# gotaku6629/CTC

Hardware: AMD Instinct MI355X
Metric: ctc_samples_per_sec (higher is better)
Workload: dtype f32; 1 GPU; NoBlankCTC B=256 T=150 C=158 S<=20 fp32 (BASELINE configs[1]); variant=noblank, per_gpu_batch=256, global_batch=256, T=150, C=158, S=20, parallelism=dp1 (batch-sharded), launch=graph, graph_steps=50, step=fused loss+grad launch + scale_grad launch (loss.backward(), grad_out=1)

## Files before the change

ctc_amd/csrc/common.hpp:

```cpp
#pragma once
#include <hip/hip_runtime.h>
#include <stdint.h>

#if !defined(CTC_AMD_EXPERIMENTS) &&                                                                            \
    (defined(CTC_X_NOSTATUS) || defined(CTC_X_NOREDUCE) || defined(CTC_X_NORETURN) || defined(CTC_X_NOCHAIN) || \
     defined(CTC_X_NOPRIO) || defined(CTC_X_NOREAD) || defined(CTC_X_NOWRITE) ||                                 \
     defined(CTC_X_WMASK) || defined(CTC_X_NOPROG) || defined(CTC_X_NORENORM) ||                                \
     defined(CTC_X_ROWDPP) || defined(CTC_X_SCALAR_STEP) || defined(CTC_X_NO_POOL_GATHER) || defined(CTC_X_FLOW_NO_GPRIO) || defined(CTC_X_FLOW_NOEXP) || defined(CTC_X_FLOW_NO_DELEGATE) || defined(CTC_X_FLOW_DELEGATE_OWN) || \
     defined(CTC_FLOW_TILE_WAVES))
#error "CTC_X_* experiment switches need -DCTC_AMD_EXPERIMENTS (A/B builds only, never the product library)"
#endif

namespace ctc {

constexpr int kWave = 64;
constexpr float kNeg = -10000000000000.0f;
constexpr float kInfeasible = 1.0e12f;

struct LaneStates { int K, SP; };
inline LaneStates lane_states(int S)
{
    int K = 1;
    while (K <= 4 && S > kWave * K) K *= 2;
    return {K, (S + K - 1) / K * K};
}

__device__ __forceinline__ int lane_id() { return threadIdx.x & (kWave - 1); }
__device__ __forceinline__ int wave_id() { return __builtin_amdgcn_readfirstlane(threadIdx.x >> 6); }

__device__ __forceinline__ void stream_store(float *p, float v) { __builtin_nontemporal_store(v, p); }
__device__ __forceinline__ void stream_store(float4 *p, float4 v)
{
    typedef float native4 __attribute__((ext_vector_type(4)));
    native4 n = {v.x, v.y, v.z, v.w};
    __builtin_nontemporal_store(n, reinterpret_cast<native4 *>(p));
}

typedef float wt_f2 __attribute__((ext_vector_type(2)));
typedef float wt_f4 __attribute__((ext_vector_type(4)));
__device__ __forceinline__ void through_store(wt_f2 *p, wt_f2 v)
{
    asm volatile("global_store_dwordx2 %0, %1, off sc1" ::"v"(p), "v"(v) : "memory");
}
__device__ __forceinline__ void through_store(wt_f4 *p, wt_f4 v)
{
    asm volatile("global_store_dwordx4 %0, %1, off sc1\n\ts_nop 1" ::"v"(p), "v"(v) : "memory");
}
typedef unsigned wt_u2 __attribute__((ext_vector_type(2)));
__device__ __forceinline__ void through_store(wt_u2 *p, wt_u2 v)
{
    asm volatile("global_store_dwordx2 %0, %1, off sc1" ::"v"(p), "v"(v) : "memory");
}
__device__ __forceinline__ void through_store(unsigned *p, unsigned v)
{
    asm volatile("global_store_dword %0, %1, off sc1" ::"v"(p), "v"(v) : "memory");
}
template <bool NT, typename V, int A = 8>
__device__ __forceinline__ void grad_store(V *p, V v)
{
    if (NT) {
        typedef V __attribute__((aligned(A))) VA;
        __builtin_nontemporal_store(v, reinterpret_cast<VA *>(p));
    } else {
        through_store(p, v);
    }
}

constexpr unsigned kStatusNoblankStarved = 1u, kStatusBinaryStarved = 2u, kStatusBlankStarved = 4u;
constexpr unsigned kStatusAlignStarved = 8u;
__device__ __forceinline__ void raise_status(unsigned *counter, unsigned bit)
{
#ifdef CTC_X_NOSTATUS
    return;
#endif
    if (lane_id() == 0) __hip_atomic_fetch_or(counter + 2, bit, __ATOMIC_RELAXED, __HIP_MEMORY_SCOPE_AGENT);
}

constexpr int kGateWord = 11;
__device__ __forceinline__ unsigned *arrival_shard(unsigned *counter, int sh) { return counter + 64 + 4 * sh + 2; }
__device__ __forceinline__ bool gate_on(const unsigned *counter)
{
    typedef const __attribute__((address_space(4))) unsigned const_u32;
    return *(const_u32 *)(uintptr_t)(counter + kGateWord) != 0;
}
__device__ __forceinline__ void note_arrival(unsigned *counter, int b)
{
    if (!gate_on(counter)) return;
    __hip_atomic_fetch_add(arrival_shard(counter, b & 15), 1u, __ATOMIC_RELAXED, __HIP_MEMORY_SCOPE_AGENT);
}
__device__ __forceinline__ void reset_arrivals(unsigned *counter)
{
    for (int sh = 0; sh < 16; ++sh) __hip_atomic_store(arrival_shard(counter, sh), 0u, __ATOMIC_RELAXED, __HIP_MEMORY_SCOPE_AGENT);
}

#ifdef CTC_AMD_DIAGNOSTICS
#define CTC_DIAG(p) ((p).stop)
#else
#define CTC_DIAG(p) 0
#endif

__device__ __forceinline__ void lds_order() { asm volatile("" ::: "memory"); }

__device__ __forceinline__ int opaque_v(int x) { asm volatile("" : "+v"(x)); return x; }
__device__ __forceinline__ int opaque_s(int x) { asm volatile("" : "+s"(x)); return x; }

__device__ __forceinline__ int xcd_sample(int bid, int B)
{
    const int x = bid & 7, k = bid >> 3, q = B >> 3, r = B & 7;
    return x * q + (x < r ? x : r) + k;
}

__device__ __forceinline__ float wave_shr1(float v, float fill)
{
    return __builtin_bit_cast(float, __builtin_amdgcn_update_dpp(
        __builtin_bit_cast(int, fill), __builtin_bit_cast(int, v), 0x138, 0xf, 0xf, false));
}
__device__ __forceinline__ float wave_shl1(float v, float fill)
// ... 299 lines not shown
```

ctc_amd/csrc/noblank.hip:

```cpp
#include <type_traits>

#include "lattice.hpp"
#include "launch.hpp"

namespace ctc {

struct NoblankParams {
    const float *x;
    int64_t st, sb;
    const void *lab;
    int lab64;
    const int64_t *in_len, *tgt_len;
    int T, B, C, S, SP;
    int stop;
    float loss_scale, grad_scale;
    float *nll, *loss, *grad;
    float *gamma;
    float *lattice;
    int64_t slab;
    unsigned *counter;
    int next_round;
    float ls_a, ls_b;
    int koff;
};
// ... 472 lines not shown
            pl.next_round = (q.B > cus && (size_t)q.T * ((q.C * 4 + 127) / 128) <= (size_t)kKmWorkers * kWave) ? cus : 0;
            return pl;
        }
#endif
        pl.family = kNoblankR16;
        pl.next_round = (q.B > cus && (size_t)q.T * ((q.C * esz + 127) / 128) <= (size_t)kPipeWorkers * kWave) ? cus : 0;
        pl.ps = q.B > 2 * cus && cus > 0 && !q.sw.no_ps && q.want_grad && 4 * n4 + 2 * n2 <= 12;
        if (pl.ps) pl.grid = cus;
        return pl;
    }
    if (r16_only || (z.glb && z.smem > kMaxLds)) return NoblankPlan{};
    if (fast) {
        pl.ch = (q.C + kWave - 1) / kWave;
        pl.dual = q.B > cus && 2 * z.smem <= kMaxLds;
        const size_t xsmem = xr_smem_bytes(q.T, z.SP, q.C);
        const bool xr = !q.sw.no_xr && xsmem <= kMaxLds && (!pl.dual || 2 * xsmem <= kMaxLds);
        pl.family = xr ? kNoblankXr : kNoblankPipelined;
        pl.lds = xr ? xsmem : z.smem;
        return pl;
    }
    pl.family = kNoblankFused;
    pl.K = z.K; pl.glb = z.glb;
    pl.ch = q.C <= 256 && !z.glb ? (q.C + kWave - 1) / kWave : 0;
    pl.lds = z.smem;
    return pl;
}

template <int N, int... Ns, typename F>
static int with_constant(int n, F f)
{
    if constexpr (sizeof...(Ns) == 0) {
        return f(std::integral_constant<int, N>());
    } else {
        return n == N ? f(std::integral_constant<int, N>()) : with_constant<Ns...>(n, f);
    }
}
template <typename F>
static int with_row_chunks(int n4, int n2, F f)
{
    return with_constant<1, 2, 4, 5, 6, 8, 9, 10, 12, 13, 14, 16>(4 * n4 + n2, [&](auto k) {
        return f(std::integral_constant<int, decltype(k)::value / 4>(), std::integral_constant<int, decltype(k)::value % 4>());
    });
}

static int noblank_launch(const NoblankPlan &pl, int dtype, NoblankParams &p, hipStream_t s)
{
    const dim3 grid(pl.grid), block(kThreads);
    p.next_round = pl.next_round; p.koff = pl.koff;
    switch (pl.family) {
        case kNoblankR16:
            return with_row_chunks(pl.n4, pl.n2, [&](auto n4, auto n2) {
                return with_constant<0, 1>(pl.nt, [&](auto nt) {
                    return with_constant<CTC_AMD_BF16, CTC_AMD_F16, CTC_AMD_F32>(dtype, [&](auto dt) {
                        using E = std::conditional_t<decltype(dt)::value == CTC_AMD_BF16, __bf16,
                                                     std::conditional_t<decltype(dt)::value == CTC_AMD_F16, _Float16, float>>;
                        constexpr int A = decltype(n4)::value, Bq = decltype(n2)::value;
                        constexpr bool NT = decltype(nt)::value != 0;
                        if constexpr (4 * A + 2 * Bq <= 12)
                            if (pl.ps) return launch<noblank_r16_kernel<A, Bq, NT, true, E>>(grid, block, pl.lds, s, p);
                        return launch<noblank_r16_kernel<A, Bq, NT, false, E>>(grid, block, pl.lds, s, p);
                    });
                });
            });
#ifdef CTC_AMD_DIAGNOSTICS
        case kNoblankKm:
            return with_row_chunks(pl.n4, pl.n2, [&](auto n4, auto n2) {
                return with_constant<0, 1>(pl.nt, [&](auto nt) {
                    return launch<noblank_km_kernel<decltype(n4)::value, decltype(n2)::value, decltype(nt)::value != 0>>(
                        grid, block, pl.lds, s, p);
                });
            });
#endif
        case kNoblankXr:
        case kNoblankPipelined:
            return with_constant<1, 2, 3, 4>(pl.ch, [&](auto ch) {
                return with_constant<0, 1>(pl.dual, [&](auto dual) {
                    constexpr int CH = decltype(ch)::value;
                    constexpr bool DUAL = decltype(dual)::value != 0;
                    return pl.family == kNoblankXr ? launch<noblank_xr_kernel<CH, DUAL>>(grid, block, pl.lds, s, p)
                                                   : launch<noblank_pipelined_kernel<CH, DUAL>>(grid, block, pl.lds, s, p);
                });
            });
        case kNoblankFused:
            return with_constant<1, 2, 4>(pl.K, [&](auto k) {
                constexpr int K = decltype(k)::value;
                if (pl.glb) return launch<noblank_fused_kernel<K, 0, true>>(grid, block, pl.lds, s, p);
                return with_constant<1, 2, 3, 4, 0>(pl.ch, [&](auto ch) {
                    return launch<noblank_fused_kernel<K, decltype(ch)::value>>(grid, block, pl.lds, s, p);
                });
            });
        default: return CTC_AMD_ERR_UNSUPPORTED_SHAPE;
    }
}

static int noblank_run(const void *x, int64_t stride_t, int64_t stride_b,
                       const void *labels, int labels_i64,
                       const int64_t *in_len, const int64_t *tgt_len,
                       int T, int B, int C, int S,
                       float loss_scale, float grad_scale,
                       float *nll, float *loss, void *grad,
                       void *workspace, void *stream, float label_smoothing, int x_dtype = CTC_AMD_F32,
                       float *gamma = nullptr)
{
    const NoblankSwitches sw = gamma ? NoblankSwitches{} : noblank_switches();
    NoblankParams p;
    if (const int rc = noblank_params(p, x, stride_t, stride_b, labels, labels_i64, in_len, tgt_len, T, B, C, S, loss_scale,
                                      grad_scale, nll, loss, grad, gamma, workspace, label_smoothing, sw))
        return rc;
    const NoblankQuery q = {T, B, C, S, x_dtype, stride_t, stride_b,
                            (unsigned)(reinterpret_cast<uintptr_t>(x) & 15), (unsigned)(reinterpret_cast<uintptr_t>(grad) & 15),
                            p.grad != nullptr, gamma != nullptr, label_smoothing >= 0.f,
                            device_cus(),
                            sw};
// ... 120 lines not shown
```

ctc_amd/csrc/noblank_km.hpp:

```cpp
#pragma once
#include "noblank_km_asm.hpp"

namespace ctc {

constexpr int kKmWorkers = 12, kKmG = 4;
constexpr int kKmPad = 8;
constexpr float kKmMinLog2 = -4096.f;
constexpr float kKmSink = -8388608.f;
constexpr float kKmNone = -16777216.f;
constexpr int kKmIntMin = -2147483647 - 1;
constexpr int kKmKprog = kKmWorkers, kKmMprog = kKmWorkers + 2;

__host__ __device__ inline int km_pitch_c(int T)
{
    int tp = T + 2 * kKmPad;
    while ((tp & 3) != 2) ++tp;
    return tp;
}
__host__ __device__ inline int km_pitch_m(int T)
{
    int tp = T + 2 * kKmPad;
    while ((tp & 7) != 4) ++tp;
    return tp;
}
// ... 603 lines not shown
        if (CTC_DIAG(p) < 0) stamp(p, 3 + (G - 1 - g) < 6 ? 3 + (G - 1 - g) : 5);
        if (first) { asm volatile("" ::"v"(prefetched)); first = false; }
        int occn[2] = {0, 0}, max_occ = 0;
        if (need_a > 0) {
            occn[0] = own[0] ? sm.occ[lst[0]] : 0;
            occn[1] = own[1] ? sm.occ[lst[1]] : 0;
            max_occ = __builtin_amdgcn_readfirstlane(sm.occ[(p.SP + 3) & ~3]);
        }
        const Row &x = v[g];
        const int t = tv[g];
        const bool live = t >= 0 && t < Tlive;
        float pr[2];
        int ks[2];
#pragma unroll
        for (int s = 0; s < 2; ++s) {
            const bool in = live && own[s];
            const int offc = in ? lst[s] * sm.TPc + t : p.SP * sm.TPc, offm = in ? lst[s] * sm.TPm + t : p.SP * sm.TPm;
            const float a = sm.ma[offm], bq = sm.mb[offm];
            const int ca = cell_k(sm.ka[offc]);
            const int kbq = __builtin_bit_cast(int, sm.kb[offc].x);
            const float pm = in ? sm.em[offc].x : 1.f;
            pr[s] = in ? a * bq * __builtin_amdgcn_rcpf(pm) : 0.f;
            ks[s] = ca + kbq;
        }
        if (__builtin_amdgcn_ballot_w64(live && !have_ref) != 0) {
            int km = max(pr[0] > 0.f ? ks[0] : kKmIntMin, pr[1] > 0.f ? ks[1] : kKmIntMin);
            row16_allmax(km);
            if (live && !have_ref && km != kKmIntMin) { kref = km; have_ref = true; }
        }
        float z[2];
#pragma unroll
        for (int s = 0; s < 2; ++s) z[s] = pr[s] > 0.f ? __builtin_amdgcn_ldexpf(pr[s], ks[s] - kref) : 0.f;
        float tot = z[0] + z[1];
        row16_allsum(tot);
        float rinv = (live && tot > 0.f) ? -gsc * p.ls_a * __builtin_amdgcn_rcpf(tot) : 0.f;
        if (starved) {
            rinv = __builtin_nanf("");
            raise_status(p.counter, kStatusNoblankStarved);
        }
        Row::zero_tile(trow, i16);
        lds_order();
#pragma unroll
        for (int s = 0; s < 2; ++s)
            if (own[s] && occn[s] == 0) *gat[s] = z[s] * rinv;
        for (int k = 1; k <= max_occ; ++k) {
            lds_order();
#pragma unroll
            for (int s = 0; s < 2; ++s)
                if (own[s] && occn[s] == k) *gat[s] += z[s] * rinv;
        }
        lds_order();
        if (t >= 0) {
            float *gp = p.grad + ((int64_t)t * p.B + b) * p.C;
            if (smooth) x.template store_grad<NT, true>(gp, trow, i16, rs[g] * (1.f - p.ls_b), col_ok, live ? -p.ls_b * gsc : 0.f);
            else x.template store_grad<NT, false>(gp, trow, i16, rs[g], col_ok, 0.f);
        }
        lds_order();
    }
    stamp(p, 7);
}

}
```

ctc_amd/csrc/noblank_r16.hpp:

```cpp
#pragma once

namespace ctc {

typedef float f2_t __attribute__((ext_vector_type(2)));

#define CTC_ROW16(OP)                                                                   \
    "s_nop 1\n\t" OP " %0, %0, %0 quad_perm:[1,0,3,2] row_mask:0xf bank_mask:0xf\n\t"   \
    "s_nop 1\n\t" OP " %0, %0, %0 quad_perm:[2,3,0,1] row_mask:0xf bank_mask:0xf\n\t"   \
    "s_nop 1\n\t" OP " %0, %0, %0 row_half_mirror row_mask:0xf bank_mask:0xf\n\t"       \
    "s_nop 1\n\t" OP " %0, %0, %0 row_mirror row_mask:0xf bank_mask:0xf\n\t"            \
    "s_nop 1"
__device__ __forceinline__ void row16_allmax(float &v) { asm volatile(CTC_ROW16("v_max_f32_dpp") : "+v"(v)); }
__device__ __forceinline__ void row16_allsum(float &v) { asm volatile(CTC_ROW16("v_add_f32_dpp") : "+v"(v)); }
__device__ __forceinline__ void row16_allmax(int &v) { asm volatile(CTC_ROW16("v_max_i32_dpp") : "+v"(v)); }

constexpr int kR16Pad = 2 * kPrefetch + 1;
#ifndef CTC_R16_BLOCK
#define CTC_R16_BLOCK 16
#endif
constexpr int kR16Block = CTC_R16_BLOCK;
__host__ __device__ inline int r16_pitch(int T)
{
    int tp = T + 2 * kR16Pad + 1;
    while ((tp & 3) != 2) ++tp;
    return tp;
}

__device__ __forceinline__ int r16_row(int T, int u, int g, int k)
{
    const int H = (T + 1) >> 1, idx = 2 * kPipeWorkers * g + 2 * u + (k >> 1);
    if ((k & 1) == 0) return idx < H ? idx : -1;
    return idx < T - H ? T - 1 - idx : -1;
}

struct R16Smem {
    int TP;
    cell_t *em, *al, *be;
    float *dummy, *stage, *cs;
    int *cnt, *lab, *occ, *done;
    __device__ R16Smem(float *base, int T, int SP, int RP)
    {
        TP = r16_pitch(T);
        cell_t *lat = reinterpret_cast<cell_t *>(base);
        em = lat + kR16Pad;
        al = em + (size_t)(SP + 1) * TP;
        be = al + (size_t)(SP + 1) * TP;
        dummy = reinterpret_cast<float *>(lat + (size_t)3 * (SP + 1) * TP);
        cnt = reinterpret_cast<int *>(dummy + 8);
        lab = cnt + 16;
        occ = lab + ((SP + 3) & ~3);
        cs = reinterpret_cast<float *>(occ + ((SP + 3) & ~3) + 4);
        done = reinterpret_cast<int *>(cs + 4 * kPipeWorkers);
        stage = cs + 64;
// ... 141 lines not shown
        if (have < G) wait_upto(i + kR16Block - 1 + kPrefetch);
        if (CTC_DIAG(p) < 0) stamp(p, 2 + i / 16);
#ifndef CTC_X_NORENORM
        renorm();
#endif
#pragma unroll
        for (int q = 0; q < kPairs; ++q) {
            const pair_t e = ring[q & 1];
#ifndef CTC_X_NOREAD
            ring[q & 1] = rb[FWD ? q : kPairs - 1 - q];
#endif
#ifdef CTC_X_NOWRITE
            const pair_t o = step2(e, q == 0);
            if (q == kPairs - 1) wb[0] = o;
#elif defined(CTC_X_WMASK)
            const pair_t o = step2(e, q == 0);
            if (lane < SP) wb[FWD ? q : kPairs - 1 - q] = o;
#else
            wb[FWD ? q : kPairs - 1 - q] = step2(e, q == 0);
#endif
        }
        rb += D * kPairs;
        wb += D * kPairs;
    }
    if (CTC_DIAG(p) == -77 && lane == 0)
        reinterpret_cast<unsigned long long *>(p.counter)[FWD ? 0 : 1] = __builtin_amdgcn_s_memtime() - loop_t0;
    lds_order();
    *prog = i;
    if (have < G) wait_upto(Tb - 1);
    renorm();
    static_assert(kPrefetch == 4, "tail groups assume one ring revolution of two pairs");
    if (!FWD) { rb += kPairs - 2; wb += kPairs - 2; }
    for (; i < Tb; i += kPrefetch) {
#pragma unroll
        for (int q = 0; q < 2; ++q) {
            const pair_t e = ring[q];
            ring[q] = rb[FWD ? q : 1 - q];
            wb[FWD ? q : 1 - q] = step2(e, q == 0);
        }
        rb += D * 2;
        wb += D * 2;
    }
    lds_order();
    *prog = Tb;
    __builtin_amdgcn_s_setprio(0);
    cell_t fin = (FWD ? sm.al : sm.be)[(size_t)(L - 1) * sm.TP + (FWD ? Tb - 1 : 0)];
    if (starved) {
        raise_status(p.counter, kStatusNoblankStarved);
        fin = make_cell(__builtin_nanf(""), 0);
    }
    return fin;
}

typedef float f4_t __attribute__((ext_vector_type(4)));
typedef float f4u_t __attribute__((ext_vector_type(4), aligned(8)));

typedef unsigned u2a4_t __attribute__((ext_vector_type(2), aligned(4)));
template <typename E>
__device__ __forceinline__ f2_t r16_widen2(unsigned u)
{
    if constexpr (__is_same(E, __bf16)) {
        const f2_t f = {__builtin_bit_cast(float, u << 16), __builtin_bit_cast(float, u & 0xffff0000u)};
        return f;
    } else {
        typedef _Float16 h2_t __attribute__((ext_vector_type(2)));
        return __builtin_convertvector(__builtin_bit_cast(h2_t, u), f2_t);
    }
}
template <typename E>
__device__ __forceinline__ unsigned r16_narrow2(f2_t v)
{
    typedef E e2_t __attribute__((ext_vector_type(2)));
    return __builtin_bit_cast(unsigned, __builtin_convertvector(v, e2_t));
}

template <bool kRaw, int N4, int N2>
struct R16RawRegs {};
template <int N4, int N2>
struct R16RawRegs<true, N4, N2> {
    wt_u2 ra[N4 > 0 ? N4 : 1];
    unsigned rc[N2 > 0 ? N2 : 1];
};

template <int N4, int N2, typename E = float>
struct R16Row : R16RawRegs<sizeof(E) == 2, N4, N2> {
    static constexpr bool kLowp = sizeof(E) == 2;
    f4_t a[N4 > 0 ? N4 : 1];
    f2_t c[N2 > 0 ? N2 : 1];
    static constexpr int kCols = 64 * N4 + 32 * N2;
    static constexpr bool kLast4 = N2 == 0;
    __device__ static __forceinline__ int off4(int j, int i16) { return 64 * j + 4 * i16; }
    __device__ static __forceinline__ int off2(int k, int i16) { return 64 * N4 + 32 * k + 2 * i16; }
    __device__ static __forceinline__ int off_last(int i16) { return kLast4 ? off4(N4 - 1, i16) : off2(N2 - 1, i16); }

    __device__ __forceinline__ void load(const E *row, int i16, int c_last)
    {
        if constexpr (kLowp) {
#pragma unroll
            for (int j = 0; j < N4; ++j)
                this->ra[j] = *reinterpret_cast<const u2a4_t *>(row + ((kLast4 && j == N4 - 1) ? c_last : off4(j, i16)));
#pragma unroll
            for (int k = 0; k < N2; ++k)
                this->rc[k] = *reinterpret_cast<const unsigned *>(row + (k == N2 - 1 ? c_last : off2(k, i16)));
        } else {
#pragma unroll
            for (int j = 0; j < N4; ++j)
// ... 37 lines not shown
            const float q = (a[j].x + a[j].y) + (a[j].z + a[j].w);
            s += ((kLast4 && j == N4 - 1) && !valid_last) ? 0.f : q;
        }
#pragma unroll
        for (int k = 0; k < N2; ++k) s += (k == N2 - 1 && !valid_last) ? 0.f : c[k].x + c[k].y;
        return s;
    }
    __device__ __forceinline__ float exp_sum(float mb, float mbl)
    {
        const f2_t l2 = {kLog2e, kLog2e};
        f2_t acc = {0.f, 0.f};
#pragma unroll
        for (int j = 0; j < N4; ++j) {
            const float b = (kLast4 && j == N4 - 1) ? mbl : mb;
            const f2_t bb = {b, b};
            f2_t lo = {a[j].x, a[j].y}, hi = {a[j].z, a[j].w};
            lo = __builtin_elementwise_fma(lo, l2, bb);
            hi = __builtin_elementwise_fma(hi, l2, bb);
            a[j].x = __builtin_amdgcn_exp2f(lo.x);
            a[j].y = __builtin_amdgcn_exp2f(lo.y);
            a[j].z = __builtin_amdgcn_exp2f(hi.x);
            a[j].w = __builtin_amdgcn_exp2f(hi.y);
            const f2_t e0 = {a[j].x, a[j].y}, e1 = {a[j].z, a[j].w};
            acc += e0;
            acc += e1;
        }
#pragma unroll
        for (int k = 0; k < N2; ++k) {
            const float b = k == N2 - 1 ? mbl : mb;
            const f2_t bb = {b, b};
            const f2_t lo = __builtin_elementwise_fma(c[k], l2, bb);
            c[k].x = __builtin_amdgcn_exp2f(lo.x);
            c[k].y = __builtin_amdgcn_exp2f(lo.y);
            acc += c[k];
        }
        return acc.x + acc.y;
    }
    __device__ __forceinline__ void to_tile(float *trow, int i16) const
    {
#pragma unroll
        for (int j = 0; j < N4; ++j) *reinterpret_cast<f4_t *>(trow + off4(j, i16)) = a[j];
#pragma unroll
        for (int k = 0; k < N2; ++k) *reinterpret_cast<f2_t *>(trow + off2(k, i16)) = c[k];
    }
    __device__ static __forceinline__ void zero_tile(float *trow, int i16)
    {
        const f4_t z4 = {0.f, 0.f, 0.f, 0.f};
        const f2_t z2 = {0.f, 0.f};
#pragma unroll
        for (int j = 0; j < N4; ++j) *reinterpret_cast<f4_t *>(trow + off4(j, i16)) = z4;
#pragma unroll
        for (int k = 0; k < N2; ++k) *reinterpret_cast<f2_t *>(trow + off2(k, i16)) = z2;
    }
    template <bool NT, bool LS>
    __device__ __forceinline__ void store_grad(E *g, const float *trow, int i16, float rs, bool col_ok, float cb) const
    {
        const f2_t r2 = {rs, rs}, cb2 = {cb, cb};
        f4_t o4[N4 > 0 ? N4 : 1];
        f2_t o2[N2 > 0 ? N2 : 1];
#pragma unroll
        for (int j = 0; j < N4; ++j) o4[j] = *reinterpret_cast<const f4_t *>(trow + off4(j, i16));
#pragma unroll
        for (int k = 0; k < N2; ++k) o2[k] = *reinterpret_cast<const f2_t *>(trow + off2(k, i16));
#pragma unroll
        for (int j = 0; j < N4; ++j) {
            const f4_t o = o4[j];
            f2_t olo = {o.x, o.y}, ohi = {o.z, o.w};
            if (LS) { olo += cb2; ohi += cb2; }
            const f2_t xlo = {a[j].x, a[j].y}, xhi = {a[j].z, a[j].w};
            const f2_t vlo = __builtin_elementwise_fma(xlo, r2, olo), vhi = __builtin_elementwise_fma(xhi, r2, ohi);
            if (!(kLast4 && j == N4 - 1) || col_ok) {
                if constexpr (kLowp) {
                    const wt_u2 n = {r16_narrow2<E>(vlo), r16_narrow2<E>(vhi)};
                    grad_store<NT, wt_u2, 4>(reinterpret_cast<wt_u2 *>(g + off4(j, i16)), n);
                } else {
                    const f4_t v = {vlo.x, vlo.y, vhi.x, vhi.y};
                    grad_store<NT>(reinterpret_cast<f4_t *>(g + off4(j, i16)), v);
                }
            }
        }
#pragma unroll
        for (int k = 0; k < N2; ++k) {
            f2_t o = o2[k];
            if (LS) o += cb2;
            const f2_t v = __builtin_elementwise_fma(c[k], r2, o);
            if (k < N2 - 1 || col_ok) {
                if constexpr (kLowp) grad_store<NT, unsigned, 4>(reinterpret_cast<unsigned *>(g + off2(k, i16)), r16_narrow2<E>(v));
                else grad_store<NT>(reinterpret_cast<f2_t *>(g + off2(k, i16)), v);
            }
        }
    }
    __device__ __forceinline__ void touch() const
    {
        if constexpr (kLowp) {
#pragma unroll
            for (int j = 0; j < N4; ++j) asm volatile("" ::"v"(this->ra[j]));
#pragma unroll
            for (int k = 0; k < N2; ++k) asm volatile("" ::"v"(this->rc[k]));
        } else {
#pragma unroll
            for (int j = 0; j < N4; ++j) asm volatile("" ::"v"(a[j]));
#pragma unroll
            for (int k = 0; k < N2; ++k) asm volatile("" ::"v"(c[k]));
        }
    }
    template <bool NT>
    __device__ static __forceinline__ void store_zero(E *g, int i16, bool col_ok)
    {
        if constexpr (kLowp) {
            const wt_u2 z4 = {0u, 0u};
#pragma unroll
            for (int j = 0; j < N4; ++j)
                if (!(kLast4 && j == N4 - 1) || col_ok) grad_store<NT, wt_u2, 4>(reinterpret_cast<wt_u2 *>(g + off4(j, i16)), z4);
#pragma unroll
            for (int k = 0; k < N2; ++k)
                if (k < N2 - 1 || col_ok) grad_store<NT, unsigned, 4>(reinterpret_cast<unsigned *>(g + off2(k, i16)), 0u);
            return;
        }
        const f4_t z4 = {0.f, 0.f, 0.f, 0.f};
        const f2_t z2 = {0.f, 0.f};
#pragma unroll
        for (int j = 0; j < N4; ++j)
            if (!(kLast4 && j == N4 - 1) || col_ok) grad_store<NT>(reinterpret_cast<f4_t *>(g + off4(j, i16)), z4);
#pragma unroll
        for (int k = 0; k < N2; ++k)
            if (k < N2 - 1 || col_ok) grad_store<NT>(reinterpret_cast<f2_t *>(g + off2(k, i16)), z2);
    }
};

static bool r16_shape(int C, int &n4, int &n2)
{
    if (C < 2 || C > 256 || (C & 1)) return false;
    const int U = (C + 31) / 32;
    if (U & 1) { n4 = U / 2; n2 = 1; }
    else if ((C & 3) == 0) { n4 = U / 2; n2 = 0; }
    else { n4 = U / 2 - 1; n2 = 2; }
    return true;
}

template <typename E>
__device__ __forceinline__ const E *r16_xrow(const NoblankParams &p, int t, int b)
{
    return reinterpret_cast<const E *>(p.x) + (int64_t)t * p.st + (int64_t)b * p.sb;
}
template <int N4, int N2, bool NT, bool PS = false, typename E = float>
__global__ __launch_bounds__(kThreads, 4) void noblank_r16_kernel(NoblankParams p)
{
    extern __shared__ float4 smem_raw[];
    typedef R16Row<N4, N2, E> Row;
    constexpr int RP = Row::kCols;
    constexpr int G = kPipeRows / 4;
    const R16Smem sm(reinterpret_cast<float *>(smem_raw), p.T, p.SP, RP);
    const int tid = threadIdx.x, w = wave_id(), lane = lane_id();
    int vb = blockIdx.x;
    int b = xcd_sample(vb, p.B);
    if (tid == 64 * kChainB) note_arrival(p.counter, b);
    const int u = (w == 0 || w == kChainB) ? -1 : (w < kChainB ? w - 1 : w - 2);
    const int rho = lane >> 4, i16 = lane & 15;

    if (CTC_DIAG(p) == 1) return;
    stamp(p, 0);
    stamp_setup(p, 0);
    auto spread = [&](int which) {
        if (CTC_DIAG(p) != -50 || w != 1 || lane != 0) return;
        const int bid = blockIdx.x, nb = gridDim.x;
        const int slot = bid == 0 ? 0 : bid == nb / 2 ? 2 : bid == nb - 1 ? 4 : -1;
        if (slot < 0) return;
        unsigned long long *o = reinterpret_cast<unsigned long long *>(p.counter) + 8 + 2 * (slot + which);
        o[0] = __builtin_amdgcn_s_memtime();
        o[1] = __builtin_amdgcn_s_memrealtime();
    };
    spread(0);
    ScalarLengths len(p.in_len + b, p.tgt_len + b);
    int tv0[G];
    Row v[G];
#ifdef CTC_R16_NX
    constexpr int NX = PS ? CTC_R16_NX : 0;
#else
    constexpr int NX = PS ? (NT ? 2 : 3) : 0;
#endif
    Row nx[NX > 0 ? NX : 1];
    const bool col_ok = Row::off_last(i16) < p.C;
    const int c_last = col_ok ? Row::off_last(i16) : p.C - (Row::kLast4 ? 4 : 2);
    const int Hh = (p.T + 1) >> 1;
    bool grp[G];
#pragma unroll
    for (int g = 0; g < G; ++g) grp[g] = u >= 0 && 2 * kPipeWorkers * g + 2 * u < Hh;
    int klab = 0;
    if (PS && w == 0 && lane < p.S) klab = load_label(p.lab, p.lab64, (int64_t)b * p.S + lane);
    if (u >= 0) {
#pragma unroll
        for (int g = 0; g < G; ++g) {
            tv0[g] = r16_row(p.T, u, g, rho);
            if (g >= NX) v[g].load(r16_xrow<E>(p, tv0[g] >= 0 ? tv0[g] : 0, b), i16, c_last);
            else nx[g].load(r16_xrow<E>(p, tv0[g] >= 0 ? tv0[g] : 0, b), i16, c_last);
        }
        stamp_setup(p, 1);
        if (PS) {
#pragma unroll
            for (int g = 0; g < G; ++g) {
// ... 43 lines not shown
        if ((vb - (int)blockIdx.x) / (int)gridDim.x < 6) stamp_mode(p, -400, (vb - (int)blockIdx.x) / (int)gridDim.x);
        return CTC_DIAG(p) != 2;
    };
    auto advance = [&]() -> bool {
        stamp_mode(p, -300, (vb - (int)blockIdx.x) / (int)gridDim.x);
        if ((vb - (int)blockIdx.x) / (int)gridDim.x < 6) stamp_mode(p, -400, 6 + (vb - (int)blockIdx.x) / (int)gridDim.x);
        if (!more) return false;
        vb = vbn;
        b = bn;
        len = len_n;
        klab = klab_n;
        asm volatile("s_waitcnt lgkmcnt(0)\n\ts_barrier" ::: "memory");
        return true;
    };
    auto chain_sample = [&](const NoblankParams &p, const int lane) {
    const R16Smem sm(reinterpret_cast<float *>(smem_raw), p.T, p.SP, RP);
    if (Tb == 0) {
        if (w == 0)
            publish_and_reduce_sum(-kNeg, b, p.B, p.nll, p.loss, p.loss_scale, p.counter);
        return;
    }
    {
        __builtin_amdgcn_s_setprio(3);
        if (w == 0) {
            const cell_t a = r16_chain<true>(p, sm, p.T, Tb, L, p.SP, lane);
            stamp(p, 11);
            bool late = false;
            {
                int spins = 0;
                while (*(lds_cvint *)sm.done < kPipeWorkers) {
                    if (++spins >= kSpinLimit) { late = true; break; }
                    __builtin_amdgcn_s_sleep(2);
                }
                lds_order();
            }
            const float csum = wave_sum(lane < 4 * kPipeWorkers ? sm.cs[lane] : 0.f);
            const float am = a.x;
            float nll = am > 0.f ? -(__builtin_amdgcn_logf(am) + (float)(cell_k(a) - kXrBias) + csum) * kLn2 : -kNeg;
            if (am != am) nll = am;
            if (late) {
                raise_status(p.counter, kStatusNoblankStarved);
                nll = __builtin_nanf("");
            }
            publish_and_reduce_sum(nll, b, p.B, p.nll, p.loss, p.loss_scale, p.counter);
            if (CTC_DIAG(p) == -50 && lane == 0) {
                const int bid = blockIdx.x, nb = gridDim.x;
                const int slot = bid == 0 ? 6 : bid == nb / 2 ? 7 : bid == nb - 1 ? 8 : -1;
                if (slot >= 0) {
                    unsigned long long *o = reinterpret_cast<unsigned long long *>(p.counter) + 8 + 2 * slot;
                    o[0] = __builtin_amdgcn_s_memtime();
                    o[1] = __builtin_amdgcn_s_memrealtime();
                }
            }
        } else if (p.grad || p.gamma) {
            r16_chain<false>(p, sm, p.T, Tb, L, p.SP, lane);
            stamp(p, 11);
        }
    }
    };

    auto worker_sample = [&](const NoblankParams &p, const int lane, const int u) {
    const R16Smem sm(reinterpret_cast<float *>(smem_raw), p.T, p.SP, RP);
    const int rho = lane >> 4, i16 = lane & 15;
    int tv[G];
#pragma unroll
    for (int g = 0; g < G; ++g) tv[g] = PS ? opaque_v(tv0[g]) : tv0[g];
    const bool has_grad = PS || p.grad != nullptr, has_gamma = !PS && !Row::kLowp && p.gamma != nullptr;
    auto load_next = [&]() {
        if (!PS) return;
#pragma unroll
        for (int g = 0; g < NX; ++g) nx[g].load(r16_xrow<E>(p, tv[g] >= 0 ? tv[g] : 0, bn), i16, c_last);
    };
#define CTC_R16_RELOAD(g)                                                                             \
    do {                                                                                              \
        if (PS && (g) >= NX) v[g].load(r16_xrow<E>(p, tv[g] >= 0 ? tv[g] : 0, bn), i16, c_last); \
    } while (0)
    if (!PS && Tb == 0) {
        if (p.grad) {
#pragma unroll
            for (int g = 0; g < G; ++g)
                if (tv[g] >= 0) Row::template store_zero<NT>(reinterpret_cast<E *>(p.grad) + ((int64_t)tv[g] * p.B + b) * p.C, i16, col_ok);
        }
        if (!Row::kLowp && p.gamma) {
#pragma unroll
            for (int g = 0; g < G; ++g)
                for (int l = i16; l < p.S && tv[g] >= 0; l += 16) p.gamma[((int64_t)b * p.T + tv[g]) * p.S + l] = 0.f;
        }
        return;
    }
    float *tile = sm.stage + (size_t)u * 4 * RP;
    float *trow = tile + rho * RP;
    int lst[2];
    float *gat[2];
#pragma unroll
    for (int s = 0; s < 2; ++s) {
        lst[s] = 16 * s + i16;
        gat[s] = trow + (lst[s] < p.SP ? sm.lab[lst[s]] : 0);
    }
    const bool own[2] = {lst[0] < L, lst[1] < L};
    const bool smooth = p.ls_b != 0.f;
    cell_t *const spare_w = reinterpret_cast<cell_t *>(sm.dummy);
    float mrow[G];
#pragma unroll
    for (int g = 0; g < G; ++g) {
        if (g == 0) __builtin_amdgcn_s_setprio(2);
        else __builtin_amdgcn_s_setprio(1);
        if (g < NX) v[g] = nx[g];
        if (grp[g]) {
            Row &x = v[g];
            x.widen();
            const int t = tv[g];
            const bool live = t >= 0 && t < Tb;
            float m = x.max();
            row16_allmax(m);
            mrow[g] = m;
            if (CTC_DIAG(p) < 0 && g == 0) stamp(p, 6);
            x.to_tile(trow, i16);
            lds_order();
            float xv[2];
#pragma unroll
            for (int s = 0; s < 2; ++s) xv[s] = *gat[s];
            lds_order();
#pragma unroll
            for (int s = 0; s < 2; ++s) {
                const float ec = (xv[s] - m) * kLog2e;
                const float e2 = fmaxf(smooth ? p.ls_a * ec : ec, kXrMinLog2);
                const float fl = __builtin_floorf(e2);
                const float pm = __builtin_amdgcn_exp2f(e2 - fl);
                cell_t *dst = (live && lst[s] < p.SP) ? sm.em + lst[s] * sm.TP + t : spare_w;
                *dst = own[s] ? make_cell(pm, (int)fl) : zero;
            }
            lds_order();
        } else {
            mrow[g] = 0.f;
        }
        sm.cnt[u] = 4 * (g + 1);
        __builtin_amdgcn_sched_barrier(0);
        if (CTC_DIAG(p) < 0) stamp(p, 8 + g);
    }
    __builtin_amdgcn_s_setprio(0);
    load_next();
    float rs[G];
    float cacc = 0.f;
#pragma unroll
    for (int g = 0; g < G; ++g) {
        rs[g] = 0.f;
        if (!grp[g]) continue;
        Row &x = v[g];
        const int t = tv[g];
        const bool live = t >= 0 && t < Tb;
        const float m = mrow[g];
        float sx = 0.f;
        if (smooth) {
            sx = x.sum(col_ok);
            row16_allsum(sx);
        }
        const float mb = -m * kLog2e;
        float sum = x.exp_sum(mb, col_ok ? mb : ninf);
        row16_allsum(sum);
        const float l2sum = __builtin_amdgcn_logf(sum);
        rs[g] = live ? p.grad_scale * __builtin_amdgcn_rcpf(sum) : 0.f;
        const float cst = smooth ? __builtin_fmaf(p.ls_b, __builtin_fmaf(sx - (float)p.C * m, kLog2e, -(float)p.C * l2sum), -p.ls_a * l2sum)
                                 : -l2sum;
        cacc += live ? cst : 0.f;
    }
    if (i16 == 0) sm.cs[4 * u + rho] = cacc;
    lds_order();
    if (lane == 0) __hip_atomic_fetch_add(sm.done, 1, __ATOMIC_RELAXED, __HIP_MEMORY_SCOPE_WORKGROUP);
    stamp(p, 2);
    if (u == kPipeWorkers - 1 && has_grad) {
        const int kl = lane < p.SP ? sm.lab[lane] : -1;
        int oc = 0;
        for (int l2 = 0; l2 < L; ++l2) {
            const int q = __builtin_amdgcn_readlane(kl, l2);
            oc += (l2 < lane && q == kl) ? 1 : 0;
        }
        if (lane >= L) oc = 0;
        int mo = 0;
        while (__builtin_amdgcn_ballot_w64(oc > mo) != 0) ++mo;
        if (lane < p.SP) sm.occ[lane] = oc;
        sm.occ[(p.SP + 3) & ~3] = mo;
        lds_order();
        sm.occ[((p.SP + 3) & ~3) + 1] = 1;
    }
    float prefetched = 0.f;
    if (!PS && p.next_round > 0 && (int)blockIdx.x + p.next_round < p.B) {
        const int nb = xcd_sample(blockIdx.x + p.next_round, p.B);
        const int line = u * kWave + lane;
        const int lines_per_row = (p.C * (int)sizeof(E) + 127) / 128;
        const int t = line / lines_per_row, c = (line - t * lines_per_row) * (128 / (int)sizeof(E));
        typedef const E __attribute__((address_space(1))) gelem;
        if (t < p.T) prefetched = (float)*(gelem *)(r16_xrow<E>(p, t, nb) + (c < p.C ? c : p.C - 1));
    }
    if (!has_grad && !has_gamma) return;

    const int Tlive = Tb;
    const float gsc = p.grad_scale;
    Row::zero_tile(trow, i16);
    lds_order();
    if (PS) {
#pragma unroll
        for (int g = 0; g < NX; ++g) nx[g].touch();
    }
    int need_a_[G], need_b_[G];
#pragma unroll
    for (int g = 0; g < G; ++g) {
        need_a_[g] = 0;
        need_b_[g] = 0;
#pragma unroll
        for (int k = 0; k < 4; ++k) {
            const int tk = r16_row(p.T, u, g, k);
            if (tk >= 0 && tk < Tlive) {
                need_a_[g] = max(need_a_[g], tk + 1);
                need_b_[g] = max(need_b_[g], Tlive - tk);
            }
        }
    }
    int crow[2];
#pragma unroll
    for (int s = 0; s < 2; ++s) crow[s] = opaque_v((lst[s] < p.SP ? lst[s] : p.SP) * sm.TP);
    E *grow[G];
#pragma unroll
    for (int g = 0; g < G; ++g) {
        grow[g] = reinterpret_cast<E *>(p.grad) + ((int64_t)(tv[g] > 0 ? tv[g] : 0) * p.B + b) * p.C;
        asm volatile("" : "+v"(grow[g]));
    }
    bool starved = false;

    int kref = 0;
    bool have_ref = false;
    int occn[2] = {0, 0}, max_occ = 0;
    if (has_grad) {
        int spins = 0;
        while (*(lds_cvint *)(sm.occ + ((p.SP + 3) & ~3) + 1) == 0) {
            if (++spins >= kSpinLimit) { starved = true; break; }
            __builtin_amdgcn_s_sleep(2);
        }
        lds_order();
        occn[0] = own[0] ? sm.occ[lst[0]] : 0;
        occn[1] = own[1] ? sm.occ[lst[1]] : 0;
        max_occ = __builtin_amdgcn_readfirstlane(sm.occ[(p.SP + 3) & ~3]);
    }
    const bool first_occ[2] = {own[0] && occn[0] == 0, own[1] && occn[1] == 0};
    float *const sink = sm.dummy + 4;
#pragma unroll
    for (int g = G - 1; g >= 0; --g) {
        if (!grp[g]) continue;
        const int need_a = need_a_[g], need_b = need_b_[g];
        if (need_a > 0) {
            int spins = 0;
            while (*(lds_cvint *)(sm.cnt + kPipeWorkers) < need_a || *(lds_cvint *)(sm.cnt + kPipeWorkers + 1) < need_b) {
                if (++spins >= kSpinLimit) { starved = true; break; }
                __builtin_amdgcn_s_sleep(8);
            }
            lds_order();
        }
#ifdef CTC_AMD_FAULT_INJECT
        if (b == 1) starved = true;
#endif
        if (CTC_DIAG(p) < 0) stamp(p, 3 + (G - 1 - g));
        if (g == G - 1) asm volatile("" ::"v"(prefetched));
        const Row &x = v[g];
        const int t = tv[g];
        const bool live = t >= 0 && t < Tlive;
        float pr[2];
        int ks[2];
#pragma unroll
        for (int s = 0; s < 2; ++s) {
            const bool in = live && own[s];
            const int off = crow[s] + (t > 0 ? t : 0);
            const cell_t a = sm.al[off], bb = sm.be[off], e = sm.em[off];
            pr[s] = in ? a.x * bb.x * __builtin_amdgcn_rcpf(e.x) : 0.f;
            ks[s] = cell_k(a) + cell_k(bb) - cell_k(e);
        }
        if (__builtin_amdgcn_ballot_w64(live && !have_ref) != 0) {
            int km = max(pr[0] > 0.f ? ks[0] : 0, pr[1] > 0.f ? ks[1] : 0);
            row16_allmax(km);
            if (live && !have_ref) { kref = km; have_ref = true; }
        }
        float z[2];
#pragma unroll
        for (int s = 0; s < 2; ++s) z[s] = __builtin_amdgcn_ldexpf(pr[s], ks[s] - kref);
        float tot = z[0] + z[1];
        row16_allsum(tot);
        if (has_gamma) {
            const float ginv = (live && tot > 0.f) ? __builtin_amdgcn_rcpf(tot) : 0.f;
#pragma unroll
            for (int s = 0; s < 2; ++s)
                if (t >= 0 && lst[s] < p.S) p.gamma[((int64_t)b * p.T + t) * p.S + lst[s]] = own[s] ? z[s] * ginv : 0.f;
            continue;
        }
        float rinv = (live && tot > 0.f) ? -gsc * p.ls_a * __builtin_amdgcn_rcpf(tot) : 0.f;
        if (starved) {
            rinv = __builtin_nanf("");
            raise_status(p.counter, kStatusNoblankStarved);
        }
#pragma unroll
        for (int s = 0; s < 2; ++s) *(first_occ[s] ? gat[s] : sink) = z[s] * rinv;
        for (int k = 1; k <= max_occ; ++k) {
            lds_order();
#pragma unroll
            for (int s = 0; s < 2; ++s)
                if (own[s] && occn[s] == k) *gat[s] += z[s] * rinv;
        }
        lds_order();
        if (t >= 0) {
            E *gp = grow[g];
            if (smooth) x.template store_grad<NT, true>(gp, trow, i16, rs[g] * (1.f - p.ls_b), col_ok, live ? -p.ls_b * gsc : 0.f);
            else x.template store_grad<NT, false>(gp, trow, i16, rs[g], col_ok, 0.f);
        }
        lds_order();
#pragma unroll
        for (int s = 0; s < 2; ++s) *(own[s] ? gat[s] : sink) = 0.f;
        lds_order();
        CTC_R16_RELOAD(g);
    }
    stamp(p, 7);
    spread(1);
#undef CTC_R16_RELOAD
    };

    if (u < 0) {
        for (;;) {
            if (!begin(true)) return;
            chain_sample(p, PS ? opaque_v(lane) : lane);
            if (!advance()) return;
        }
    }
    for (;;) {
        if (!begin(false)) return;
        if (PS) worker_sample(p, opaque_v(lane), opaque_s(u));
        else worker_sample(p, lane, u);
        if (!advance()) return;
    }
}

#ifdef CTC_AMD_DIAGNOSTICS
__global__ __launch_bounds__(kThreads, 4) void r16_chain_probe_kernel(NoblankParams p, unsigned long long *out, int waves_alive,
                                                                     int mode, int chain_b)
{
    extern __shared__ float4 smem_raw[];
    const R16Smem sm(reinterpret_cast<float *>(smem_raw), p.T, p.SP, 160);
    const int tid = threadIdx.x, w = wave_id(), lane = lane_id();
    for (int i = tid; i < 3 * (p.SP + 1) * sm.TP; i += kThreads) sm.em[i - kR16Pad] = make_cell(1.5f, -1);
    if (tid < 16) sm.cnt[tid] = kPipeRows;
    __syncthreads();
    if (w >= waves_alive && w != chain_b) return;
    if (w != 0 && w != chain_b) {
        typedef const volatile __attribute__((address_space(3))) int lds_cvint;
        int spins = 0;
        const int u = (w < chain_b ? w - 1 : w - 2) % kPipeWorkers;
        float *tile = sm.stage + (size_t)u * 4 * 160 + (lane >> 4) * 160 + 4 * (lane & 15);
        const cell_t *cells = sm.al + (size_t)(lane & 15) * sm.TP;
        if (mode & 8) __builtin_amdgcn_s_setprio(2);
        float a0 = lane, a1 = 1.f, a2 = 2.f, a3 = 3.f, acc = 0.f;
        const int kind = mode & 7;
        while (*(lds_cvint *)(sm.cnt + kPipeWorkers) < p.T && ++spins < 100000) {
            if (kind == 0) { __builtin_amdgcn_s_sleep(8); continue; }
            if (kind & 1) {
#pragma unroll
                for (int r = 0; r < 16; ++r) {
                    a0 = __builtin_fmaf(a0, 1.0001f, a1); a1 = __builtin_fmaf(a1, 0.9999f, a2);
                    a2 = __builtin_fmaf(a2, 1.0001f, a3); a3 = __builtin_fmaf(a3, 0.9999f, a0);
                    a0 = __builtin_fmaf(a0, 0.5f, a2); a1 = __builtin_fmaf(a1, 0.5f, a3);
                    a2 = __builtin_fmaf(a2, 0.5f, 1.f);
                    a3 = __builtin_amdgcn_exp2f(a3 * 1e-3f);
                }
            }
            if (kind & 2) {
                const int reps = kind == 2 ? 12 : 1;
                for (int r = 0; r < reps; ++r) {
                    f4_t v4 = {a0, a1, a2, a3};
// ... 26 lines not shown
```

Before: 19.23 million samples/s.

## Specialize r16 noblank kernel by mode and use immediate-offset gradient stores

Adds a compile-time MODE template parameter (grad, smoothed grad, gamma, forward) to the r16 kernel so the runtime checks on grad, gamma and label smoothing become constants. Gradient stores now use one base pointer per row with immediate instruction offsets instead of computing an address per chunk. The two progress counters are read in one 64-bit LDS load and made wave-uniform via readfirstlane. Starvation handling and the scale factors are hoisted out of the per-group loop. The intent is to cut scalar/vector instruction count and register pressure in the gradient phase, at the cost of more kernel instantiations.

Measured after the change: 18.65 million samples/s. 3.0% lower.

```diff
diff --git a/ctc_amd/csrc/common.hpp b/ctc_amd/csrc/common.hpp
--- a/ctc_amd/csrc/common.hpp
+++ b/ctc_amd/csrc/common.hpp
@@ -55,6 +55,26 @@
 {
     asm volatile("global_store_dword %0, %1, off sc1" ::"v"(p), "v"(v) : "memory");
 }
+template <int OFF>
+__device__ __forceinline__ void through_store_at(wt_f2 *p, wt_f2 v)
+{
+    asm volatile("global_store_dwordx2 %0, %1, off offset:%2 sc1" ::"v"(p), "v"(v), "n"(OFF) : "memory");
+}
+template <int OFF>
+__device__ __forceinline__ void through_store_at(wt_f4 *p, wt_f4 v)
+{
+    asm volatile("global_store_dwordx4 %0, %1, off offset:%2 sc1\n\ts_nop 1" ::"v"(p), "v"(v), "n"(OFF) : "memory");
+}
+template <int OFF>
+__device__ __forceinline__ void through_store_at(wt_u2 *p, wt_u2 v)
+{
+    asm volatile("global_store_dwordx2 %0, %1, off offset:%2 sc1" ::"v"(p), "v"(v), "n"(OFF) : "memory");
+}
+template <int OFF>
+__device__ __forceinline__ void through_store_at(unsigned *p, unsigned v)
+{
+    asm volatile("global_store_dword %0, %1, off offset:%2 sc1" ::"v"(p), "v"(v), "n"(OFF) : "memory");
+}
 template <bool NT, typename V, int A = 8>
 __device__ __forceinline__ void grad_store(V *p, V v)
 {
@@ -63,6 +83,17 @@
         __builtin_nontemporal_store(v, reinterpret_cast<VA *>(p));
     } else {
         through_store(p, v);
+    }
+}
+template <bool NT, int OFF, typename V, int A = 8>
+__device__ __forceinline__ void grad_store_at(V *p, V v)
+{
+    static_assert(OFF >= 0 && OFF < 4096 && OFF % A == 0, "immediate offset of a global store");
+    if (NT) {
+        typedef V __attribute__((aligned(A))) VA;
+        __builtin_nontemporal_store(v, reinterpret_cast<VA *>(reinterpret_cast<char *>(p) + OFF));
+    } else {
+        through_store_at<OFF>(p, v);
     }
 }
 
diff --git a/ctc_amd/csrc/noblank.hip b/ctc_amd/csrc/noblank.hip
--- a/ctc_amd/csrc/noblank.hip
+++ b/ctc_amd/csrc/noblank.hip
@@ -548,13 +548,18 @@
             return with_row_chunks(pl.n4, pl.n2, [&](auto n4, auto n2) {
                 return with_constant<0, 1>(pl.nt, [&](auto nt) {
                     return with_constant<CTC_AMD_BF16, CTC_AMD_F16, CTC_AMD_F32>(dtype, [&](auto dt) {
-                        using E = std::conditional_t<decltype(dt)::value == CTC_AMD_BF16, __bf16,
-                                                     std::conditional_t<decltype(dt)::value == CTC_AMD_F16, _Float16, float>>;
-                        constexpr int A = decltype(n4)::value, Bq = decltype(n2)::value;
-                        constexpr bool NT = decltype(nt)::value != 0;
-                        if constexpr (4 * A + 2 * Bq <= 12)
-                            if (pl.ps) return launch<noblank_r16_kernel<A, Bq, NT, true, E>>(grid, block, pl.lds, s, p);
-                        return launch<noblank_r16_kernel<A, Bq, NT, false, E>>(grid, block, pl.lds, s, p);
+                        const int mode = p.gamma ? kR16Gamma : !p.grad ? kR16Fwd : p.ls_b != 0.f ? kR16GradSmooth : kR16Grad;
+                        return with_constant<kR16Grad, kR16GradSmooth, kR16Gamma, kR16Fwd>(mode, [&](auto md) {
+                            using E = std::conditional_t<decltype(dt)::value == CTC_AMD_BF16, __bf16,
+                                                         std::conditional_t<decltype(dt)::value == CTC_AMD_F16, _Float16, float>>;
+                            constexpr int A = decltype(n4)::value, Bq = decltype(n2)::value;
+                            constexpr int MD = sizeof(E) == 2 ? (int)kR16Runtime : decltype(md)::value;
+                            constexpr bool kGradMode = MD == kR16Grad || MD == kR16GradSmooth || MD == kR16Runtime;
+                            constexpr bool NT = decltype(nt)::value != 0 && kGradMode;
+                            if constexpr (4 * A + 2 * Bq <= 12 && kGradMode)
+                                if (pl.ps) return launch<noblank_r16_kernel<A, Bq, NT, true, E, MD>>(grid, block, pl.lds, s, p);
+                            return launch<noblank_r16_kernel<A, Bq, NT, false, E, MD>>(grid, block, pl.lds, s, p);
+                        });
                     });
                 });
             });
diff --git a/ctc_amd/csrc/noblank_km.hpp b/ctc_amd/csrc/noblank_km.hpp
--- a/ctc_amd/csrc/noblank_km.hpp
+++ b/ctc_amd/csrc/noblank_km.hpp
@@ -679,8 +679,8 @@
         lds_order();
         if (t >= 0) {
             float *gp = p.grad + ((int64_t)t * p.B + b) * p.C;
-            if (smooth) x.template store_grad<NT, true>(gp, trow, i16, rs[g] * (1.f - p.ls_b), col_ok, live ? -p.ls_b * gsc : 0.f);
-            else x.template store_grad<NT, false>(gp, trow, i16, rs[g], col_ok, 0.f);
+            if (smooth) x.template store_grad<NT, true>(Row::grad_base4(gp, i16), Row::grad_base2(gp, i16), trow, i16, rs[g] * (1.f - p.ls_b), col_ok, live ? -p.ls_b * gsc : 0.f);
+            else x.template store_grad<NT, false>(Row::grad_base4(gp, i16), Row::grad_base2(gp, i16), trow, i16, rs[g], col_ok, 0.f);
         }
         lds_order();
     }
diff --git a/ctc_amd/csrc/noblank_r16.hpp b/ctc_amd/csrc/noblank_r16.hpp
--- a/ctc_amd/csrc/noblank_r16.hpp
+++ b/ctc_amd/csrc/noblank_r16.hpp
@@ -1,4 +1,6 @@
 #pragma once
+
+#include <utility>
 
 namespace ctc {
 
@@ -246,6 +248,11 @@
     return fin;
 }
 
+template <int N, typename F, int... Is>
+__device__ __forceinline__ void r16_static_for_(F &&f, std::integer_sequence<int, Is...>) { (f(std::integral_constant<int, Is>()), ...); }
+template <int N, typename F>
+__device__ __forceinline__ void r16_static_for(F &&f) { r16_static_for_<N>(f, std::make_integer_sequence<int, N>()); }
+
 typedef float f4_t __attribute__((ext_vector_type(4)));
 typedef float f4u_t __attribute__((ext_vector_type(4), aligned(8)));
 
@@ -389,9 +396,12 @@
 #pragma unroll
         for (int k = 0; k < N2; ++k) *reinterpret_cast<f2_t *>(trow + off2(k, i16)) = z2;
     }
+    __device__ static __forceinline__ E *grad_base4(E *row, int i16) { return row + off4(0, i16); }
+    __device__ static __forceinline__ E *grad_base2(E *row, int i16) { return row + (off2(0, i16) - off2(0, 0)); }
     template <bool NT, bool LS>
-    __device__ __forceinline__ void store_grad(E *g, const float *trow, int i16, float rs, bool col_ok, float cb) const
-    {
+    __device__ __forceinline__ void store_grad(E *g4, E *g2, const float *trow, int i16, float rs, bool col_ok, float cb) const
+    {
+        constexpr int kE = (int)sizeof(E);
         const f2_t r2 = {rs, rs}, cb2 = {cb, cb};
         f4_t o4[N4 > 0 ? N4 : 1];
         f2_t o2[N2 > 0 ? N2 : 1];
@@ -399,8 +409,8 @@
         for (int j = 0; j < N4; ++j) o4[j] = *reinterpret_cast<const f4_t *>(trow + off4(j, i16));
 #pragma unroll
         for (int k = 0; k < N2; ++k) o2[k] = *reinterpret_cast<const f2_t *>(trow + off2(k, i16));
-#pragma unroll
-        for (int j = 0; j < N4; ++j) {
+        r16_static_for<N4>([&](auto jc) {
+            constexpr int j = decltype(jc)::value;
             const f4_t o = o4[j];
             f2_t olo = {o.x, o.y}, ohi = {o.z, o.w};
             if (LS) { olo += cb2; ohi += cb2; }
@@ -409,23 +419,23 @@
             if (!(kLast4 && j == N4 - 1) || col_ok) {
                 if constexpr (kLowp) {
                     const wt_u2 n = {r16_narrow2<E>(vlo), r16_narrow2<E>(vhi)};
-                    grad_store<NT, wt_u2, 4>(reinterpret_cast<wt_u2 *>(g + off4(j, i16)), n);
+                    grad_store_at<NT, 64 * j * kE, wt_u2, 4>(reinterpret_cast<wt_u2 *>(g4), n);
                 } else {
                     const f4_t v = {vlo.x, vlo.y, vhi.x, vhi.y};
-                    grad_store<NT>(reinterpret_cast<f4_t *>(g + off4(j, i16)), v);
+                    grad_store_at<NT, 64 * j * kE>(reinterpret_cast<f4_t *>(g4), v);
                 }
             }
-        }
-#pragma unroll
-        for (int k = 0; k < N2; ++k) {
+        });
+        r16_static_for<N2>([&](auto kc) {
+            constexpr int k = decltype(kc)::value;
             f2_t o = o2[k];
             if (LS) o += cb2;
             const f2_t v = __builtin_elementwise_fma(c[k], r2, o);
             if (k < N2 - 1 || col_ok) {
-                if constexpr (kLowp) grad_store<NT, unsigned, 4>(reinterpret_cast<unsigned *>(g + off2(k, i16)), r16_narrow2<E>(v));
-                else grad_store<NT>(reinterpret_cast<f2_t *>(g + off2(k, i16)), v);
-            }
-        }
+                if constexpr (kLowp) grad_store_at<NT, (64 * N4 + 32 * k) * kE, unsigned, 4>(reinterpret_cast<unsigned *>(g2), r16_narrow2<E>(v));
+                else grad_store_at<NT, (64 * N4 + 32 * k) * kE>(reinterpret_cast<f2_t *>(g2), v);
+            }
+        });
     }
     __device__ __forceinline__ void touch() const
     {
@@ -480,9 +490,13 @@
 {
     return reinterpret_cast<const E *>(p.x) + (int64_t)t * p.st + (int64_t)b * p.sb;
 }
-template <int N4, int N2, bool NT, bool PS = false, typename E = float>
+enum R16Mode { kR16Grad = 0, kR16GradSmooth = 1, kR16Gamma = 2, kR16Fwd = 3, kR16Runtime = 4 };
+template <int N4, int N2, bool NT, bool PS = false, typename E = float, int MODE = kR16Runtime>
 __global__ __launch_bounds__(kThreads, 4) void noblank_r16_kernel(NoblankParams p)
 {
+    static_assert(!PS || MODE == kR16Grad || MODE == kR16GradSmooth || MODE == kR16Runtime, "persistent form: gradient launches only");
+    static_assert(!(sizeof(E) == 2 && MODE == kR16Gamma), "posteriors: fp32 logits only");
+    constexpr bool kRt = MODE == kR16Runtime;
     extern __shared__ float4 smem_raw[];
     typedef R16Row<N4, N2, E> Row;
     constexpr int RP = Row::kCols;
@@ -632,7 +646,7 @@
                     o[1] = __builtin_amdgcn_s_memrealtime();
                 }
             }
-        } else if (p.grad || p.gamma) {
+        } else if (kRt ? (p.grad || p.gamma) : MODE != kR16Fwd) {
             r16_chain<false>(p, sm, p.T, Tb, L, p.SP, lane);
             stamp(p, 11);
         }
@@ -645,23 +659,29 @@
     int tv[G];
 #pragma unroll
     for (int g = 0; g < G; ++g) tv[g] = PS ? opaque_v(tv0[g]) : tv0[g];
-    const bool has_grad = PS || p.grad != nullptr, has_gamma = !PS && !Row::kLowp && p.gamma != nullptr;
+    const bool has_grad = kRt ? (PS || p.grad != nullptr) : (MODE == kR16Grad || MODE == kR16GradSmooth);
+    const bool has_gamma = kRt ? (!PS && !Row::kLowp && p.gamma != nullptr) : MODE == kR16Gamma;
     auto load_next = [&]() {
         if (!PS) return;
 #pragma unroll
         for (int g = 0; g < NX; ++g) nx[g].load(r16_xrow<E>(p, tv[g] >= 0 ? tv[g] : 0, bn), i16, c_last);
     };
+#ifdef CTC_R16_MARKERS
+#define CTC_R16_MARK(g) asm volatile("; r16 P3 group %0" ::"n"(g))
+#else
+#define CTC_R16_MARK(g) do { } while (0)
+#endif
 #define CTC_R16_RELOAD(g)                                                                             \
     do {                                                                                              \
         if (PS && (g) >= NX) v[g].load(r16_xrow<E>(p, tv[g] >= 0 ? tv[g] : 0, bn), i16, c_last); \
     } while (0)
     if (!PS && Tb == 0) {
-        if (p.grad) {
+        if (has_grad) {
 #pragma unroll
             for (int g = 0; g < G; ++g)
                 if (tv[g] >= 0) Row::template store_zero<NT>(reinterpret_cast<E *>(p.grad) + ((int64_t)tv[g] * p.B + b) * p.C, i16, col_ok);
         }
-        if (!Row::kLowp && p.gamma) {
+        if (has_gamma) {
 #pragma unroll
             for (int g = 0; g < G; ++g)
                 for (int l = i16; l < p.S && tv[g] >= 0; l += 16) p.gamma[((int64_t)b * p.T + tv[g]) * p.S + l] = 0.f;
@@ -678,7 +698,7 @@
         gat[s] = trow + (lst[s] < p.SP ? sm.lab[lst[s]] : 0);
     }
     const bool own[2] = {lst[0] < L, lst[1] < L};
-    const bool smooth = p.ls_b != 0.f;
+    const bool smooth = (kRt || MODE == kR16Fwd) ? p.ls_b != 0.f : MODE == kR16GradSmooth;
     cell_t *const spare_w = reinterpret_cast<cell_t *>(sm.dummy);
     float mrow[G];
 #pragma unroll
@@ -740,6 +760,7 @@
         row16_allsum(sum);
         const float l2sum = __builtin_amdgcn_logf(sum);
         rs[g] = live ? p.grad_scale * __builtin_amdgcn_rcpf(sum) : 0.f;
+        if (smooth) rs[g] *= 1.f - p.ls_b;
         const float cst = smooth ? __builtin_fmaf(p.ls_b, __builtin_fmaf(sx - (float)p.C * m, kLog2e, -(float)p.C * l2sum), -p.ls_a * l2sum)
                                  : -l2sum;
         cacc += live ? cst : 0.f;
@@ -782,30 +803,40 @@
 #pragma unroll
         for (int g = 0; g < NX; ++g) nx[g].touch();
     }
-    int need_a_[G], need_b_[G];
+    int need_[G];
 #pragma unroll
     for (int g = 0; g < G; ++g) {
-        need_a_[g] = 0;
-        need_b_[g] = 0;
+        int na = 0, nb = 0;
 #pragma unroll
         for (int k = 0; k < 4; ++k) {
             const int tk = r16_row(p.T, u, g, k);
             if (tk >= 0 && tk < Tlive) {
-                need_a_[g] = max(need_a_[g], tk + 1);
-                need_b_[g] = max(need_b_[g], Tlive - tk);
-            }
-        }
+                na = max(na, tk + 1);
+                nb = max(nb, Tlive - tk);
+            }
+        }
+        need_[g] = opaque_s(na | (nb << 16));
     }
     int crow[2];
 #pragma unroll
     for (int s = 0; s < 2; ++s) crow[s] = opaque_v((lst[s] < p.SP ? lst[s] : p.SP) * sm.TP);
-    E *grow[G];
+    E *grow4[G], *grow2[G];
 #pragma unroll
     for (int g = 0; g < G; ++g) {
-        grow[g] = reinterpret_cast<E *>(p.grad) + ((int64_t)(tv[g] > 0 ? tv[g] : 0) * p.B + b) * p.C;
-        asm volatile("" : "+v"(grow[g]));
-    }
+        E *row = reinterpret_cast<E *>(p.grad) + ((int64_t)(tv[g] > 0 ? tv[g] : 0) * p.B + b) * p.C;
+        grow4[g] = Row::grad_base4(row, i16);
+        grow2[g] = Row::grad_base2(row, i16);
+        if (N4 > 0) asm volatile("" : "+v"(grow4[g]));
+        if (N2 > 0) asm volatile("" : "+v"(grow2[g]));
+    }
+    float occ_scale = smooth ? -gsc * p.ls_a : -gsc, occ_dead = 0.f;
+    const float ls_cb = smooth ? -p.ls_b * gsc : 0.f;
+    asm volatile("" : "+v"(occ_scale));
     bool starved = false;
+    auto starve = [&]() {
+        starved = true;
+        occ_scale = occ_dead = __builtin_nanf("");
+    };
 
     int kref = 0;
     bool have_ref = false;
@@ -813,7 +844,7 @@
     if (has_grad) {
         int spins = 0;
         while (*(lds_cvint *)(sm.occ + ((p.SP + 3) & ~3) + 1) == 0) {
-            if (++spins >= kSpinLimit) { starved = true; break; }
+            if (++spins >= kSpinLimit) { starve(); break; }
             __builtin_amdgcn_s_sleep(2);
         }
         lds_order();
@@ -823,20 +854,29 @@
     }
     const bool first_occ[2] = {own[0] && occn[0] == 0, own[1] && occn[1] == 0};
     float *const sink = sm.dummy + 4;
+    typedef const volatile __attribute__((address_space(3))) unsigned long long lds_cvu64;
+    const int *const progress = sm.cnt + kPipeWorkers;
 #pragma unroll
     for (int g = G - 1; g >= 0; --g) {
         if (!grp[g]) continue;
-        const int need_a = need_a_[g], need_b = need_b_[g];
-        if (need_a > 0) {
+        CTC_R16_MARK(g);
+        if (need_[g] != 0) {
+            const int need_a = need_[g] & 0xffff, need_b = need_[g] >> 16;
             int spins = 0;
-            while (*(lds_cvint *)(sm.cnt + kPipeWorkers) < need_a || *(lds_cvint *)(sm.cnt + kPipeWorkers + 1) < need_b) {
-                if (++spins >= kSpinLimit) { starved = true; break; }
+            bool ready;
+            for (;;) {
+                const unsigned long long pg = *(lds_cvu64 *)progress;
+                const int pa = __builtin_amdgcn_readfirstlane((int)(unsigned)pg);
+                const int pb = __builtin_amdgcn_readfirstlane((int)(unsigned)(pg >> 32));
+                ready = ((pa - need_a) | (pb - need_b)) >= 0;
+                if (ready || ++spins >= kSpinLimit) break;
                 __builtin_amdgcn_s_sleep(8);
             }
+            if (!ready) starve();
             lds_order();
         }
 #ifdef CTC_AMD_FAULT_INJECT
-        if (b == 1) starved = true;
+        if (b == 1) starve();
 #endif
         if (CTC_DIAG(p) < 0) stamp(p, 3 + (G - 1 - g));
         if (g == G - 1) asm volatile("" ::"v"(prefetched));
@@ -870,11 +910,7 @@
                 if (t >= 0 && lst[s] < p.S) p.gamma[((int64_t)b * p.T + t) * p.S + lst[s]] = own[s] ? z[s] * ginv : 0.f;
             continue;
         }
-        float rinv = (live && tot > 0.f) ? -gsc * p.ls_a * __builtin_amdgcn_rcpf(tot) : 0.f;
-        if (starved) {
-            rinv = __builtin_nanf("");
-            raise_status(p.counter, kStatusNoblankStarved);
-        }
+        const float rinv = (live && tot > 0.f) ? occ_scale * __builtin_amdgcn_rcpf(tot) : occ_dead;
 #pragma unroll
         for (int s = 0; s < 2; ++s) *(first_occ[s] ? gat[s] : sink) = z[s] * rinv;
         for (int k = 1; k <= max_occ; ++k) {
@@ -885,9 +921,8 @@
         }
         lds_order();
         if (t >= 0) {
-            E *gp = grow[g];
-            if (smooth) x.template store_grad<NT, true>(gp, trow, i16, rs[g] * (1.f - p.ls_b), col_ok, live ? -p.ls_b * gsc : 0.f);
-            else x.template store_grad<NT, false>(gp, trow, i16, rs[g], col_ok, 0.f);
+            if (smooth) x.template store_grad<NT, true>(grow4[g], grow2[g], trow, i16, rs[g], col_ok, live ? ls_cb : 0.f);
+            else x.template store_grad<NT, false>(grow4[g], grow2[g], trow, i16, rs[g], col_ok, 0.f);
         }
         lds_order();
 #pragma unroll
@@ -895,9 +930,12 @@
         lds_order();
         CTC_R16_RELOAD(g);
     }
+    CTC_R16_MARK(-1);
+    if (starved && !has_gamma) raise_status(p.counter, kStatusNoblankStarved);
     stamp(p, 7);
     spread(1);
 #undef CTC_R16_RELOAD
+#undef CTC_R16_MARK
     };
 
     if (u < 0) {
```
